# davrempe/caspr

Hardware: AMD Instinct MI355X
Metric: sequences/sec (CaSPR.reconstruct, rigid-cars T=10 N=2048) (higher is better)
Workload: dtype f32 (operands split exactly into 3 bf16, 6 bf16-MFMA partial products per product, f32 accumulate)

## Files before the change

caspr_amd/config.py:

```python
import os
import warnings
from dataclasses import dataclass, asdict


@dataclass
class KernelConfig:
    matmul: str = "bf16x6"
    cnf_split: str = "f16x3"
    cnf_dp5_split: str = "bf16x6"
    conv_split: str = "f16x3"
    emd_route: str = "frame"
    conv_x6w: bool = True
    x6w_min_cin: int = 512
    latent_team: bool = True
    early_latent: bool = True
    early_latent_team: bool = True
    sa_lo_parts: bool = True
    sa_scale_streams: bool = True
    global_stream: bool = True
    sa_pre_aggregate: bool = True
    fp_commute: bool = True
    sa_f64_streams: bool = False
    train_cnf_out_node: bool = True
    train_cnf_hidden_node: bool = True
    train_latent_node: bool = True
    train_cnf_checkpoint: bool = False
    train_cnf_block_node: bool = False


_ENV = {
    "CASPR_MATMUL": ("matmul", lambda v: v.strip().lower()),
    "CASPR_CNF_SPLIT": ("cnf_split", lambda v: v.strip().lower()),
    "CASPR_CNF_DP5_SPLIT": ("cnf_dp5_split", lambda v: v.strip().lower()),
    "CASPR_CONV_SPLIT": ("conv_split", lambda v: v.strip().lower()),
    "CASPR_EMD_ROUTE": ("emd_route", lambda v: v.strip().lower()),
    "CASPR_CONV_X6W": ("conv_x6w", lambda v: v != "0"),
    "CASPR_X6W_MIN_CIN": ("x6w_min_cin", int),
    "CASPR_LATENT_TEAM": ("latent_team", lambda v: v != "0"),
    "CASPR_EARLY_LATENT": (None, None),
    "CASPR_SA_LO_PARTS": ("sa_lo_parts", lambda v: v != "0"),
    "CASPR_SA_SCALE_STREAMS": ("sa_scale_streams", lambda v: v != "0"),
    "CASPR_SA_F64_STREAMS": ("sa_f64_streams", lambda v: v != "0"),
    "CASPR_FP_COMMUTE": ("fp_commute", lambda v: v != "0"),
    "CASPR_SA_PRE_AGGREGATE": ("sa_pre_aggregate", lambda v: v != "0"),
    "CASPR_GLOBAL_STREAM": ("global_stream", lambda v: v != "0"),
    "CASPR_CNF_OUT_NODE": ("train_cnf_out_node", lambda v: v != "0"),
    "CASPR_CNF_NODE": ("train_cnf_hidden_node", lambda v: v != "0"),
    "CASPR_LATENT_NODE": ("train_latent_node", lambda v: v != "0"),
    "CASPR_CNF_CHECKPOINT": ("train_cnf_checkpoint", lambda v: v != "0"),
    "CASPR_CNF_BLOCK_NODE": ("train_cnf_block_node", lambda v: v != "0"),
}


def load(environ=None):
    env = os.environ if environ is None else environ
    cfg = KernelConfig()
    present = [k for k in _ENV if k in env]
    if env.get("CASPR_DEBUG", "0") != "1":
# ... 8 lines not shown
            cfg.early_latent_team = env[name] != "single"
        else:
            setattr(cfg, field, parse(env[name]))
    if cfg.matmul not in ("bf16x6", "f32"):
        raise ValueError("CASPR_MATMUL must be 'bf16x6' or 'f32', got %r" % cfg.matmul)
    if cfg.cnf_split not in ("bf16x6", "f16x3"):
        raise ValueError("CASPR_CNF_SPLIT must be 'bf16x6' or 'f16x3', got %r" % cfg.cnf_split)
    if cfg.cnf_dp5_split not in ("bf16x6", "f16x3"):
        raise ValueError("CASPR_CNF_DP5_SPLIT must be 'bf16x6' or 'f16x3', got %r" % cfg.cnf_dp5_split)
    if cfg.conv_split not in ("bf16x6", "f16x3"):
        raise ValueError("CASPR_CONV_SPLIT must be 'bf16x6' or 'f16x3', got %r" % cfg.conv_split)
    if cfg.emd_route not in ("frame", "rows"):
        raise ValueError("CASPR_EMD_ROUTE must be 'frame' or 'rows', got %r" % cfg.emd_route)
    return cfg


config = load()


def active():
    from . import ops
    from .models import caspr as _c, pointnet2 as _p, tpointnet2 as _t
    d = asdict(config)
    d.update({"matmul": ops.matmul_mode(), "cnf_split": ops.CNF_SPLIT, "cnf_dp5_split": ops.CNF_DP5_SPLIT, "conv_split": ops.CONV_SPLIT, "emd_route": ops.EMD_ROUTE, "conv_x6w": ops.CONV_X6W, "x6w_min_cin": ops._X6W_MIN_CIN, "latent_team": ops.LATENT_TEAM,
              "early_latent": _c.EARLY_LATENT, "early_latent_team": _c.EARLY_LATENT_TEAM, "sa_lo_parts": _p.LO_PARTS,
              "sa_scale_streams": _p.SCALE_STREAMS, "sa_f64_streams": _p.F64_STREAMS, "fp_commute": _p.FP_COMMUTE, "sa_pre_aggregate": _p.PRE_AGGREGATE, "global_stream": _t.GLOBAL_STREAM, "debug_env": os.environ.get("CASPR_DEBUG", "0") == "1"})
    return d
```

caspr_amd/csrc/audit.py:

```python
import os
import re
import subprocess
import tempfile

LLVM = os.environ.get("CASPR_LLVM_BIN", "/opt/rocm/lib/llvm/bin")
TESTED_HIPCC = "HIP version: 7.2.26015-fc0010cf6a / AMD clang version 22.0.0git roc-7.2.0"


class AuditError(RuntimeError):
    pass


def tools_present():
    return all(os.path.exists(os.path.join(LLVM, t)) for t in ("llvm-objdump", "llvm-objcopy", "llvm-readelf", "clang-offload-bundler"))


def _code_object(obj):
    with tempfile.TemporaryDirectory() as d:
        fat, elf = os.path.join(d, "w.fatbin"), os.path.join(d, "w.elf")
        subprocess.check_call([os.path.join(LLVM, "llvm-objcopy"), "--dump-section", ".hip_fatbin=" + fat, obj, os.path.join(d, "copy.o")])
        subprocess.check_call([os.path.join(LLVM, "clang-offload-bundler"), "--unbundle", "--type=o", "--input=" + fat,
                               "--targets=hipv4-amdgcn-amd-amdhsa--gfx950", "--output=" + elf])
        notes = subprocess.check_output([os.path.join(LLVM, "llvm-readelf"), "--notes", elf], text=True)
        dis = subprocess.check_output([os.path.join(LLVM, "llvm-objdump"), "-d", elf], text=True)
# ... 119 lines not shown
        mfma = [i for i in ins if i.startswith("v_mfma")]
        _need(len(mfma) == 2 * 192 and all(re.match(r"v_mfma_f32_32x32x16_bf16 a\[", i) for i in mfma), "%s: %d MFMAs, not all on a[..]" % (k, len(mfma)))
        out.append({"kernel": k, "accvgpr_reads": r, "accvgpr_writes": w, "mfma": len(mfma)})
    return out


def audit_conv_h3w(obj):
    notes, dis = _code_object(obj)
    kernels = re.findall(r"<(_Z18conv1x1_h3w_kernelI[^>]*)>:", dis)
    _need(len(kernels) >= 4, "conv1x1_h3w_kernel: %d instantiations found" % len(kernels))
    out = []
    for k in kernels:
        meta, ins = _kernel(notes, dis, k)
        count = lambda pat: sum(1 for i in ins if re.match(pat, i))
        _no_spills(meta, ins, k)
        r, w = count(r"v_accvgpr_read_b32"), count(r"v_accvgpr_write_b32")
        _need(w == 768 and r == 512 and count(r"v_accvgpr_mov") == 0, "%s: %d reads / %d writes of the accumulator file (512 / 768 in the source)" % (k, r, w))
        mfma = [i for i in ins if i.startswith("v_mfma")]
        _need(len(mfma) == 2 * 96 and all(re.match(r"v_mfma_f32_32x32x16_f16 a\[", i) for i in mfma), "%s: %d MFMAs, not all v_mfma_f32_32x32x16_f16 on a[..]" % (k, len(mfma)))
        out.append({"kernel": k, "accvgpr_reads": r, "accvgpr_writes": w, "mfma": len(mfma), "cvt_pk": count(r"v_cvt_pk_f16_f32")})
    return out


AUDITS = {"ode_bf16x6w.hip": audit_cnf_x6w, "ode_f16x3w.hip": audit_cnf_h3w, "ode_dp5_f16x3w.hip": audit_cnf_dp5_h3w, "gemm_bf16x6w.hip": audit_conv_x6w, "gemm_f16x3w.hip": audit_conv_h3w}


def audit_objects(objs_by_source):
    if not tools_present():
        raise AuditError("the ROCm LLVM tools (%s: llvm-objdump, llvm-objcopy, llvm-readelf, clang-offload-bundler) are needed to audit the "
                         "hand-managed accumulator kernels" % LLVM)
    res = {}
    for src, fn in AUDITS.items():
        if src in objs_by_source:
            try:
                res[src] = fn(objs_by_source[src])
            except (AuditError, ValueError, IndexError, subprocess.CalledProcessError) as e:
                ver = subprocess.run([os.environ.get("HIPCC", "/opt/rocm/bin/hipcc"), "--version"], capture_output=True, text=True).stdout.splitlines()[:2]
                raise AuditError("%s\n  this compiler: %s\n  tested with:   %s\n  -> the library is NOT produced (CASPR_SKIP_AUDIT=1 overrides, "
                                 "see caspr_amd/csrc/audit.py)" % (e, " / ".join(ver), TESTED_HIPCC)) from None
    return res


def audit_no_packed_f32(objs_by_source):
    if not tools_present():
        raise AuditError("the ROCm LLVM tools (%s) are needed to check the objects for packed-f32 instructions" % LLVM)
    res = {}
    for src, obj in sorted(objs_by_source.items()):
# ... 11 lines not shown
```

caspr_amd/csrc/build.py:

```python
import os
import subprocess
import sys
from concurrent.futures import ThreadPoolExecutor

HERE = os.path.dirname(os.path.abspath(__file__))
sys.path.insert(0, os.path.abspath(os.path.join(HERE, "..", "..")))
SOURCES = ["point_ops.hip", "gemm.hip", "gemm_bf16x6.hip", "gemm_bf16x6w.hip", "gemm_f16x3w.hip", "sa_mlp.hip", "ode.hip", "ode_bf16x6.hip", "ode_bf16x6w.hip", "ode_f16x3w.hip", "cnf_frame_steps.hip", "ode_dp5.hip", "ode_dp5_f16x3w.hip", "ode_train_fwd.hip", "ode_sample_tape.hip", "ode_latent_dp5.hip", "backward.hip", "backward_points.hip", "backward_flow.hip", "backward_flow_value.hip", "emd.hip", "emd_exact.hip", "pose.hip", "base_sample.hip"]
EXTRA = {"point_ops.hip": ["-ffp-contract=off"], "emd.hip": ["-ffp-contract=off"], "pose.hip": ["-ffp-contract=off"],
         "emd_exact.hip": ["-ffp-contract=off"],
         "cnf_frame_steps.hip": ["-ffp-contract=off"],
         "base_sample.hip": ["-ffp-contract=off"],
         "ode_bf16x6.hip": ["-mllvm", "-pragma-unroll-threshold=400000"],
         "ode_dp5.hip": ["-mllvm", "-pragma-unroll-threshold=400000"],
         "ode_train_fwd.hip": ["-mllvm", "-pragma-unroll-threshold=400000"],
         "ode_sample_tape.hip": ["-mllvm", "-pragma-unroll-threshold=400000"],
         "ode_bf16x6w.hip": ["-mllvm", "-pragma-unroll-threshold=400000", "-mllvm", "-amdgpu-mfma-vgpr-form", "-fno-slp-vectorize"],
         "ode_f16x3w.hip": ["-mllvm", "-pragma-unroll-threshold=400000", "-mllvm", "-amdgpu-mfma-vgpr-form", "-fno-slp-vectorize"],
         "ode_dp5_f16x3w.hip": ["-mllvm", "-pragma-unroll-threshold=400000", "-mllvm", "-amdgpu-mfma-vgpr-form", "-fno-slp-vectorize"],
         "gemm_bf16x6w.hip": ["-mllvm", "-pragma-unroll-threshold=400000", "-mllvm", "-amdgpu-mfma-vgpr-form", "-fno-slp-vectorize"],
         "gemm_f16x3w.hip": ["-mllvm", "-pragma-unroll-threshold=400000", "-mllvm", "-amdgpu-mfma-vgpr-form", "-fno-slp-vectorize"]}
DEBUG = os.environ.get("CASPR_BUILD_DEBUG", "0") not in ("0", "")
XW_EXP = os.environ.get("CASPR_XW_EXP", "")
DEBUG = DEBUG or bool(XW_EXP)
OUT = os.path.join(HERE, ("libcaspr_hip_debug_xw%s.so" % XW_EXP) if XW_EXP else ("libcaspr_hip_debug.so" if DEBUG else "libcaspr_hip.so"))
HIPCC = os.environ.get("HIPCC", "/opt/rocm/bin/hipcc")
NO_PACKED_F32 = ["-Xclang", "-target-feature", "-Xclang", "-packed-fp32-ops"]
FLAGS = ["--offload-arch=gfx950", "-O3", "-std=c++17", "-fPIC", "-Wall", "-Wno-unused-function"] + NO_PACKED_F32


def _stale(target, deps):
    if not os.path.exists(target):
        return True
    t = os.path.getmtime(target)
    return any(os.path.getmtime(d) > t for d in deps)


def deps():
    inc = os.path.join(HERE, "..", "..", "include")
    return [os.path.abspath(__file__)] + sorted(os.path.join(HERE, f) for f in os.listdir(HERE) if f.endswith((".h", ".inc"))) + sorted(os.path.join(inc, f) for f in os.listdir(inc) if f.endswith(".h"))


def build(force=False, verbose=False):
# ... 41 lines not shown
```

caspr_amd/csrc/gemm_bf16x6.hip:

```cpp
#include "common.h"
#include <type_traits>

typedef short bf16x8 __attribute__((ext_vector_type(8)));
typedef unsigned u32x4 __attribute__((ext_vector_type(4)));

#define X6_TM 256
#define X6_TP 128
#define X6_PA (X6_TM * 64)
#define X6_PB (X6_TP * 64)
#define X6_CHUNK (3 * X6_PA)
#define X6_LDS (3 * X6_PA + 3 * X6_PB)

__device__ __host__ __forceinline__ int x6_swz(int row) { return (row >> 1) & 3; }
__device__ __forceinline__ int x6_off(int row, int piece) { return row * 64 + ((piece ^ x6_swz(row)) << 4); }

__device__ __forceinline__ void x6_split(float x, float &h1, float &h2, float &h3)
{
    h1 = __uint_as_float(__float_as_uint(x) & 0xffff0000u);
    const float r1 = x - h1;
    h2 = __uint_as_float(__float_as_uint(r1) & 0xffff0000u);
    const float r2 = r1 - h2;
    h3 = __uint_as_float(__float_as_uint(r2) & 0xffff0000u);
}
typedef __bf16 x6_bf16x2 __attribute__((ext_vector_type(2)));
// ... 676 lines not shown
                                  X6Act{gate, const_cast<float *>(Z), ldz, (float *)ws});
    if (rc != CASPR_OK) return rc;
    const long tot = (long)frames * Cout;
    cnf_act_bwd_reduce_kernel<<<dim3((unsigned)((tot + 255) / 256)), dim3(256), 0, (hipStream_t)stream>>>((const float *)ws, frames, 2 * n / X6_TP * 2, Cout,
                                                                                                         dgate, dbeta);
    CASPR_CHECK_LAUNCH("conv1x1_cnf_act_bwd");
    return CASPR_OK;
}

extern "C" int caspr_conv1x1_bf16x6_f32(const void *wpk, const float *bias, const float *bbias, const float *X, int ldx,
                                        const float *in_scale, const float *in_shift, int in_relu, int in_relu_from, float *Y,
                                        int ldy, int B, int P, int Cin, int Cout, int act, void *stream)
{
    CASPR_REQUIRE(Y, "conv1x1_bf16x6: Y is NULL");
    return conv_x6_launch(wpk, bias, bbias, X, ldx, in_scale, in_shift, in_relu, in_relu_from, Y, ldy, B, P, Cin, Cout, act, nullptr, stream);
}

extern "C" long caspr_conv_gn_ws_bytes(int B, int P, int Cout)
{
    if (B <= 0 || P <= 0 || Cout <= 0 || P % X6_TP) return 0;
    return (long)B * (P / X6_TP) * Cout * 16;
}

static int conv_gn_x6_impl(const void *wpk, const float *bias, const float *bbias, const float *X, int ldx, const float *in_scale,
                           const float *in_shift, int in_relu, int in_relu_from, float *Y, int ldy, int B, int P, int Cin, int Cout, int G,
                           int pool, const float *gamma, const float *beta, float eps, float *scale, float *shift, float *pmax, float *mean,
                           float *rstd, void *ws, long ws_bytes, void *stream)
{
    CASPR_REQUIRE(gamma && beta && scale && shift && ws && G > 0, "conv1x1_gn_bf16x6: bad arguments");
    CASPR_REQUIRE(Cout % G == 0, "conv1x1_gn_bf16x6: Cout=%d is not a multiple of the %d groups", Cout, G);
    CASPR_REQUIRE((mean == nullptr) == (rstd == nullptr), "conv1x1_gn_bf16x6: mean / rstd must be given together");
    CASPR_REQUIRE(pool >= 1 && B % pool == 0, "conv1x1_gn_bf16x6: pool=%d must divide B=%d", pool, B);
    CASPR_REQUIRE(B <= 65535 * (long)pool, "conv1x1_gn_bf16x6: B too large");
    CASPR_REQUIRE(P % X6_TP == 0 && ws_bytes >= caspr_conv_gn_ws_bytes(B, P, Cout) && ((uintptr_t)ws % 16) == 0,
                  "conv1x1_gn_bf16x6: workspace too small or misaligned (%ld < %ld)", ws_bytes, caspr_conv_gn_ws_bytes(B, P, Cout));
    const int rc = conv_x6_launch(wpk, bias, bbias, X, ldx, in_scale, in_shift, in_relu, in_relu_from, Y, ldy, B, P, Cin, Cout, 0,
                                  (f32x4 *)ws, stream);
    if (rc != CASPR_OK) return rc;
    conv_gn_finalize_kernel<<<dim3(G, B / pool), dim3(256), 0, (hipStream_t)stream>>>((const f32x4 *)ws, pool * (P / X6_TP), pool * P, Cout, G, gamma,
                                                                                      beta, eps, scale, shift, pmax, mean, rstd);
    CASPR_CHECK_LAUNCH("conv1x1_gn_bf16x6");
    return CASPR_OK;
}

extern "C" int caspr_conv1x1_gn_bf16x6_f32(const void *wpk, const float *bias, const float *bbias, const float *X, int ldx,
                                           const float *in_scale, const float *in_shift, int in_relu, int in_relu_from, float *Y,
                                           int ldy, int B, int P, int Cin, int Cout, int G, const float *gamma, const float *beta,
                                           float eps, float *scale, float *shift, float *pmax, float *mean, float *rstd, void *ws,
                                           long ws_bytes, void *stream)
{
    return conv_gn_x6_impl(wpk, bias, bbias, X, ldx, in_scale, in_shift, in_relu, in_relu_from, Y, ldy, B, P, Cin, Cout, G, 1, gamma, beta, eps, scale,
                           shift, pmax, mean, rstd, ws, ws_bytes, stream);
}

extern "C" int caspr_conv1x1_gn_pooled_bf16x6_f32(const void *wpk, const float *bias, const float *bbias, const float *X, int ldx,
                                                  const float *in_scale, const float *in_shift, int in_relu, int in_relu_from, float *Y,
                                                  int ldy, int B, int P, int Cin, int Cout, int G, int pool, const float *gamma,
                                                  const float *beta, float eps, float *scale, float *shift, float *pmax, float *mean,
                                                  float *rstd, void *ws, long ws_bytes, void *stream)
{
// ... 196 lines not shown
```

caspr_amd/lib.py:

```python
import ctypes
import os

_HERE = os.path.dirname(os.path.abspath(__file__))
SO_PATH = os.path.join(_HERE, "csrc", "libcaspr_hip.so")

c_fp = ctypes.c_void_p
c_ip = ctypes.c_void_p
c_int = ctypes.c_int
c_long = ctypes.c_long
c_float = ctypes.c_float
c_stream = ctypes.c_void_p

SIGNATURES = {
    "caspr_last_error_string": (ctypes.c_char_p, []),
    "caspr_abi_version": (c_int, []),
    "caspr_prep_input_f32": (c_int, [c_fp, c_int, c_int, c_int, c_int, c_fp, c_fp, c_stream]),
    "caspr_fps_f32": (c_int, [c_fp, c_int, c_int, c_int, c_int, c_ip, c_fp, c_stream]),
    "caspr_gather_points_f32": (c_int, [c_fp, c_int, c_ip, c_int, c_int, c_int, c_int, c_fp, c_int, c_stream]),
    "caspr_ball_query_f32": (c_int, [c_fp, c_fp, c_int, c_int, c_int, c_float, c_int, c_ip, c_stream]),
    "caspr_ball_query2_f32": (c_int, [c_fp, c_fp, c_int, c_int, c_int, c_float, c_int, c_ip, c_float, c_int, c_ip, c_stream]),
    "caspr_group_points_f32": (c_int, [c_fp, c_fp, c_fp, c_int, c_ip, c_int, c_int, c_int, c_int, c_int, c_fp, c_stream]),
    "caspr_sa_mlp_max_f32": (c_int, [c_fp, c_fp, c_fp, c_int, c_ip, c_int, c_int, c_int, c_int, c_int, c_int,
                                     c_fp, c_fp, c_fp, c_fp, c_int,
                                     c_fp, c_fp, c_fp, c_fp, c_int,
# ... 3 lines not shown
    "caspr_sa_mlp_max_ws_f32": (c_int, [c_fp, c_fp, c_fp, c_int, c_ip, c_int, c_int, c_int, c_int, c_int, c_int,
                                        c_fp, c_fp, c_fp, c_fp, c_int,
                                        c_fp, c_fp, c_fp, c_fp, c_int,
                                        c_fp, c_fp, c_fp, c_fp, c_int,
                                        c_fp, c_int, c_int, c_ip, c_stream]),
    "caspr_sa_mlp_max_pre_f32": (c_int, [c_fp, c_fp, c_fp, c_int, c_ip, c_int, c_int, c_int, c_int,
                                         c_fp, c_fp, c_fp, c_fp, c_int,
                                         c_fp, c_fp, c_fp, c_fp, c_int,
                                         c_fp, c_fp, c_fp, c_fp, c_int,
                                         c_fp, c_int, c_int, c_stream]),
    "caspr_group_rows_pre_f32": (c_int, [c_fp, c_fp, c_fp, c_int, c_ip, c_int, c_int, c_int, c_int, c_int, c_fp, c_fp, c_fp, c_int, c_stream]),
    "caspr_three_nn_f32": (c_int, [c_fp, c_fp, c_int, c_int, c_int, c_fp, c_ip, c_fp, c_stream]),
    "caspr_three_interp_f32": (c_int, [c_fp, c_int, c_ip, c_fp, c_fp, c_fp, c_int, c_fp, c_int, c_int, c_int, c_int, c_int, c_int, c_fp, c_int, c_stream]),
    "caspr_three_interp_add_gn_ws_bytes": (c_long, [c_int, c_int, c_int]),
    "caspr_three_interp_add_gn_f32": (c_int, [c_fp, c_int, c_ip, c_fp, c_fp, c_int, c_int, c_fp, c_fp, c_int, c_int, c_int, c_int, c_fp, c_int,
                                              c_int, c_fp, c_fp, c_float, c_fp, c_fp, ctypes.c_void_p, c_long, c_stream]),
    "caspr_packed_size": (c_long, [c_int, c_int]),
    "caspr_pack_weight_f32": (c_int, [c_fp, c_int, c_int, c_int, c_int, c_fp, c_stream]),
    "caspr_conv1x1_f32": (c_int, [c_fp, c_fp, c_fp, c_fp, c_int, c_fp, c_fp, c_int, c_int, c_fp, c_int, c_int, c_int, c_int, c_int, c_int, c_stream]),
    "caspr_bf16x3_packed_bytes": (c_long, [c_int, c_int]),
    "caspr_pack_weight_bf16x3": (c_int, [c_fp, c_int, c_int, c_int, c_int, ctypes.c_void_p, c_stream]),
    "caspr_conv1x1_bf16x6_f32": (c_int, [ctypes.c_void_p, c_fp, c_fp, c_fp, c_int, c_fp, c_fp, c_int, c_int, c_fp, c_int, c_int, c_int, c_int, c_int, c_int, c_stream]),
    "caspr_conv_gn_ws_bytes": (c_long, [c_int, c_int, c_int]),
    "caspr_conv1x1_gn_bf16x6_f32": (c_int, [ctypes.c_void_p, c_fp, c_fp, c_fp, c_int, c_fp, c_fp, c_int, c_int, c_fp, c_int, c_int, c_int, c_int, c_int,
                                            c_int, c_fp, c_fp, c_float, c_fp, c_fp, c_fp, c_fp, c_fp, ctypes.c_void_p, c_long, c_stream]),
    "caspr_conv1x1_gn_pooled_bf16x6_f32": (c_int, [ctypes.c_void_p, c_fp, c_fp, c_fp, c_int, c_fp, c_fp, c_int, c_int, c_fp, c_int, c_int, c_int, c_int, c_int,
                                                   c_int, c_int, c_fp, c_fp, c_float, c_fp, c_fp, c_fp, c_fp, c_fp, ctypes.c_void_p, c_long, c_stream]),
    "caspr_x6w_packed_bytes": (c_long, [c_int, c_int]),
    "caspr_pack_weight_x6w": (c_int, [c_fp, c_int, c_int, c_int, c_int, ctypes.c_void_p, c_stream]),
    "caspr_conv1x1_x6w_f32": (c_int, [ctypes.c_void_p, ctypes.c_void_p, c_fp, c_fp, c_fp, c_int, c_fp, c_fp, c_int, c_int, c_fp, c_int, c_int, c_int, c_int,
                                      c_int, c_int, c_fp, c_fp, c_float, c_fp, c_fp, c_fp, c_fp, c_fp, ctypes.c_void_p, c_long, c_stream]),
    "caspr_conv1x1_x6w_pooled_f32": (c_int, [ctypes.c_void_p, ctypes.c_void_p, c_fp, c_fp, c_fp, c_int, c_fp, c_fp, c_int, c_int, c_fp, c_int, c_int, c_int, c_int,
                                             c_int, c_int, c_int, c_fp, c_fp, c_float, c_fp, c_fp, c_fp, c_fp, c_fp, ctypes.c_void_p, c_long, c_stream]),
    "caspr_conv1x1_x6w_part_f32": (c_int, [ctypes.c_void_p, ctypes.c_void_p, c_fp, c_fp, c_fp, c_int, c_fp, c_fp, c_int, c_int, c_fp, c_int, c_int, c_int, c_int,
                                           c_int, c_int, c_int, c_int, c_int, ctypes.c_void_p, c_long, c_stream]),
    "caspr_h3w_packed_bytes": (c_long, [c_int, c_int]),
    "caspr_pack_weight_h3w": (c_int, [c_fp, c_int, c_int, c_int, c_int, ctypes.c_void_p, c_stream]),
    "caspr_conv1x1_h3w_f32": (c_int, [ctypes.c_void_p, ctypes.c_void_p, c_fp, c_fp, c_fp, c_int, c_fp, c_fp, c_int, c_int, c_fp, c_int, c_int, c_int, c_int,
                                      c_int, c_int, c_fp, c_fp, c_float, c_fp, c_fp, c_fp, c_fp, c_fp, ctypes.c_void_p, c_long, ctypes.c_void_p, c_stream]),
    "caspr_conv1x1_h3w_pooled_f32": (c_int, [ctypes.c_void_p, ctypes.c_void_p, c_fp, c_fp, c_fp, c_int, c_fp, c_fp, c_int, c_int, c_fp, c_int, c_int, c_int, c_int,
                                             c_int, c_int, c_int, c_fp, c_fp, c_float, c_fp, c_fp, c_fp, c_fp, c_fp, ctypes.c_void_p, c_long, ctypes.c_void_p,
                                             c_stream]),
    "caspr_conv1x1_h3w_part_f32": (c_int, [ctypes.c_void_p, ctypes.c_void_p, c_fp, c_fp, c_fp, c_int, c_fp, c_fp, c_int, c_int, c_fp, c_int, c_int, c_int, c_int,
                                           c_int, c_int, c_int, c_int, c_int, ctypes.c_void_p, c_long, ctypes.c_void_p, c_stream]),
    "caspr_conv_gn_finalize_f32": (c_int, [ctypes.c_void_p, c_long, c_int, c_int, c_int, c_int, c_int, c_int, c_int, c_fp, c_fp, c_float, c_fp, c_fp, c_fp, c_fp,
                                           c_fp, c_stream]),
# ... 134 lines not shown
```

caspr_amd/ops.py:

```python
import contextlib
import ctypes
import functools

import torch

from . import lib as _lib
from .config import config as _cfg


TIMING = False
TIMERS = {}
TIMING_ONLY = None


class timed:

    def __init__(self, name, level=1):
        self.name = name
        self.level = level

    def __enter__(self):
        self.on = TIMING >= self.level and (TIMING_ONLY is None or TIMING != True or self.name in TIMING_ONLY)
        if self.on:
            self.t0 = torch.cuda.Event(enable_timing=True)
# ... 170 lines not shown
    n = idx.shape[1]
    C = gamma.numel()
    C2 = 0 if skip is None else int(skip_channels)
    y = torch.empty(B, n, C, device=u.device, dtype=torch.float32)
    scale = torch.empty(B, C, device=u.device, dtype=torch.float32)
    shift = torch.empty(B, C, device=u.device, dtype=torch.float32)
    L = _lib.load()
    nb = L.caspr_three_interp_add_gn_ws_bytes(B, n, groups)
    ws = _workspace(nb, u.device)
    with timed("k:three_interp_add_gn:%d:%d:%d" % (C2, C, B * n), 2):
        _lib.check(L.caspr_three_interp_add_gn_f32(_p(u), ldu, _p(idx), _p(weight), _p(skip), lds, C2, _p(wskip), _p(bias), B, m, n, C, _p(y), C,
                                                   groups, _p(gamma), _p(beta), float(eps), _p(scale), _p(shift), _p(ws), ws.numel(), _stream()),
                   "caspr_three_interp_add_gn_f32")
    return y, scale, shift


_mode = _cfg.matmul
CONV_BF16X6 = _mode == "bf16x6"
CONV_X6W = _cfg.conv_x6w
CNF_BF16X6 = _mode == "bf16x6"
CNF_SPLIT = _cfg.cnf_split
CNF_DP5_SPLIT = _cfg.cnf_dp5_split

CONV_SPLIT = _cfg.conv_split


def _split_switch(name):
    value = globals()[name]
    if value not in ("bf16x6", "f16x3"):
        raise ValueError("caspr_amd.ops.%s must be 'bf16x6' or 'f16x3', got %r" % (name, value))
    return value


def conv_split():
    return _split_switch("CONV_SPLIT")


def cnf_dp5_split():
    return _split_switch("CNF_DP5_SPLIT")


def cnf_split():
    return _split_switch("CNF_SPLIT")


_X6_MIN_CIN = 192
# ... 79 lines not shown
        if self._xh is None:
            w2d, ldw, col0, version = self._src
            if w2d._version != version:
                raise RuntimeError("PackedWeight.xh(): the weight tensor was modified in place after this pack was built")
            L = _lib.load()
            cmain = self.cout - self.cout % 512
            main = torch.empty(L.caspr_h3w_packed_bytes(cmain, self.cin), device=w2d.device, dtype=torch.uint8)
            _lib.check(L.caspr_pack_weight_h3w(_p(w2d), ldw, cmain, col0, self.cin, _p(main), _stream()), "caspr_pack_weight_h3w")
            tail = None
            if cmain != self.cout:
                if self._xw is not None:
                    tail = self._xw[1]
                else:
                    wt = w2d[cmain:]
                    tail = torch.empty(L.caspr_bf16x3_packed_bytes(self.cout - cmain, self.cin), device=w2d.device, dtype=torch.uint8)
                    _lib.check(L.caspr_pack_weight_bf16x3(_p(wt), ldw, self.cout - cmain, col0, self.cin, _p(tail), _stream()), "caspr_pack_weight_bf16x3")
            self._xh = (main, tail)
            if self._x3 is not None and self._xw is not None:
                self._src = None
        return self._xh


CONV_ROW_INVARIANT = 0x100


def _pinned(n, dtype):
    return torch.empty(n, dtype=dtype).pin_memory()


def _copy_behind(host, src, stream=None):
    ev = torch.cuda.Event()
    if stream is None:
        host.copy_(src, non_blocking=True)
        ev.record(torch.cuda.current_stream())
    else:
        with torch.cuda.stream(stream):
            host.copy_(src, non_blocking=True)
            ev.record(stream)
    return ev


class _Deferred:
    BACKLOG = 64

    def __init__(self, report):
        self.report = report
# ... 255 lines not shown
    return (y, scale, shift) + (() if mean is None else (mean, rstd)) + (() if pmax is None else (pmax,))


def conv1x1_gn(pw, bias, x, gamma, beta, groups=16, eps=1e-5, want_max=False, want_moments=False, write=True, bbias=None,
               in_scale=None, in_shift=None, in_relu=False, in_relu_from=0, out=None, pool=1, split=None):
    _chk_f32(bias, bbias, in_scale, in_shift, gamma, beta)
    B, P, _ = x.shape
    C = pw.cout
    if pool < 1 or B % pool:
        raise ValueError("conv1x1_gn: pool=%d must divide the %d batch entries" % (pool, B))
    route = _conv_route(pw, B, P, in_relu_from, groups=groups, split=split)
    if route is None:
        y = conv1x1(pw, bias, x, bbias=bbias, in_scale=in_scale, in_shift=in_shift, in_relu=in_relu, in_relu_from=in_relu_from, out=out, split=split)
        yg = y.view(B // pool, pool * P, y.shape[2]) if pool > 1 else y
        if want_moments:
            from . import train_ops
            return (y,) + tuple(train_ops.gn_stats_train(yg, C, gamma, beta, groups, eps, want_max))
        return (y,) + tuple(gn_stats(yg, C, gamma, beta, groups, eps, want_max))
    ldx = _conv_ldx("conv1x1_gn", pw, x)
    y, ldy, scale, shift, mean, rstd, pmax, ws = _conv_gn_buffers(pw, x, pool, groups if want_moments else 0, want_max, out, write)
    if split is None:
        conv_split()
    packs = _conv_wide_packs(route, pw)
    with timed(_conv_timer(route, pw, x), 2):
        _conv_launch(route, "pooled" if pool > 1 else "gn", pw, packs, x, _conv_head(pw, bias, bbias, x, ldx, in_scale, in_shift, in_relu, in_relu_from, y, ldy),
                     (groups,) + ((int(pool),) if pool > 1 else ()) + (_p(gamma), _p(beta), float(eps), _p(scale), _p(shift), _p(pmax), _p(mean), _p(rstd),
                                                                       _p(ws), ws.numel()))
    return _conv_gn_result(y, scale, shift, mean, rstd, pmax)


def _conv_part(route, pw, packs, x, head, ws, mt0, mt1, with_tail, reserve):
    _conv_launch(route, "part", pw, packs, x, head, (mt0, mt1, int(with_tail), int(reserve), _p(ws), ws.numel()))


def _conv_gn_finalize(ws, x, C, groups, pool, gamma, beta, eps, scale, shift, pmax, g0, g1):
    _lib.check(_lib.load().caspr_conv_gn_finalize_f32(_p(ws), ws.numel(), x.shape[0], x.shape[1], C, groups, g0, g1, int(pool), _p(gamma), _p(beta),
                                                      float(eps), _p(scale), _p(shift), _p(pmax), None, None, _stream()), "caspr_conv_gn_finalize_f32")


def conv1x1_gn_early_ok(pw, B, P, groups, early_channels):
    C = pw.cout
    return bool(_conv_route(pw, B, P) in _CONV_WIDE and C % groups == 0 and C // 512 >= 2 and early_channels <= min(C // groups, 512))


def conv1x1_gn_early(pw, bias, x, gamma, beta, on_early, groups=16, eps=1e-5, in_scale=None, in_shift=None, in_relu=False, in_relu_from=0,
                     reserve_cus=1, tail_stream=None):
    _chk_f32(bias, in_scale, in_shift, gamma, beta)
    B, P, _ = x.shape
# ... 727 lines not shown
```

include/caspr_hip.h:

```cpp
#ifndef CASPR_HIP_H
#define CASPR_HIP_H

#include <stdint.h>

#ifdef __cplusplus
extern "C" {
#endif

#define CASPR_OK 0
#define CASPR_EINVAL (-1)
#define CASPR_ELAUNCH (-2)
#define CASPR_EUNSUP (-3)
#define CASPR_ENOCONV (-4)

const char *caspr_last_error_string(void);
int caspr_abi_version(void);

int caspr_prep_input_f32(const float *x, int BT, int N, int quad, int pairs, float *xyz, float *feat,
                         void *stream);

int caspr_fps_f32(const float *xyz, int B, int n, int M, int guard, int32_t *idx, float *new_xyz,
                  void *stream);

int caspr_gather_points_f32(const float *feat, int ldf, const int32_t *idx, int B, int n, int M, int C,
// ... 44 lines not shown
                           const float *in_scale, const float *in_shift, int in_relu, const float *skip,
                           int lds, int B, int m, int n, int C, int C2, float *out, int ldo, void *stream);
long caspr_three_interp_add_gn_ws_bytes(int B, int n, int G);
int caspr_three_interp_add_gn_f32(const float *u, int ldu, const int32_t *idx, const float *weight, const float *skip, int lds,
                                  int C2, const float *wskip, const float *bias, int B, int m, int n, int C, float *y, int ldy,
                                  int G, const float *gamma, const float *beta, float eps, float *scale, float *shift, void *ws,
                                  long ws_bytes, void *stream);


long caspr_packed_size(int Cout, int Cin);
int caspr_pack_weight_f32(const float *w, int ldw, int Cout, int col0, int ncols, float *packed,
                          void *stream);
#define CASPR_CONV_ROW_INVARIANT 0x100
int caspr_conv1x1_f32(const float *wp, const float *bias, const float *bbias, const float *X, int ldx,
                      const float *in_scale, const float *in_shift, int in_relu, int in_relu_from,
                      float *Y, int ldy, int B, int P, int Cin, int Cout, int act, void *stream);

long caspr_bf16x3_packed_bytes(int Cout, int Cin);
int caspr_pack_weight_bf16x3(const float *w, int ldw, int Cout, int col0, int ncols, void *packed, void *stream);
int caspr_conv1x1_bf16x6_f32(const void *wpk, const float *bias, const float *bbias, const float *X, int ldx,
                             const float *in_scale, const float *in_shift, int in_relu, int in_relu_from,
                             float *Y, int ldy, int B, int P, int Cin, int Cout, int act, void *stream);

long caspr_conv_gn_ws_bytes(int B, int P, int Cout);
int caspr_conv1x1_gn_bf16x6_f32(const void *wpk, const float *bias, const float *bbias, const float *X, int ldx,
                                const float *in_scale, const float *in_shift, int in_relu, int in_relu_from,
                                float *Y, int ldy, int B, int P, int Cin, int Cout, int G, const float *gamma,
                                const float *beta, float eps, float *scale, float *shift, float *pmax, float *mean,
                                float *rstd, void *ws, long ws_bytes, void *stream);
int caspr_conv1x1_gn_pooled_bf16x6_f32(const void *wpk, const float *bias, const float *bbias, const float *X, int ldx,
                                       const float *in_scale, const float *in_shift, int in_relu, int in_relu_from,
                                       float *Y, int ldy, int B, int P, int Cin, int Cout, int G, int pool,
                                       const float *gamma, const float *beta, float eps, float *scale, float *shift,
                                       float *pmax, float *mean, float *rstd, void *ws, long ws_bytes, void *stream);

long caspr_x6w_packed_bytes(int Cout, int Cin);
int caspr_pack_weight_x6w(const float *w, int ldw, int Cout, int col0, int ncols, void *packed, void *stream);
int caspr_conv1x1_x6w_f32(const void *wpk_main, const void *wpk_tail, const float *bias, const float *bbias, const float *X, int ldx,
                          const float *in_scale, const float *in_shift, int in_relu, int in_relu_from, float *Y, int ldy, int B,
                          int P, int Cin, int Cout, int G, const float *gamma, const float *beta, float eps, float *scale,
                          float *shift, float *pmax, float *mean, float *rstd, void *ws, long ws_bytes, void *stream);
int caspr_conv1x1_x6w_pooled_f32(const void *wpk_main, const void *wpk_tail, const float *bias, const float *bbias, const float *X, int ldx,
                                 const float *in_scale, const float *in_shift, int in_relu, int in_relu_from, float *Y, int ldy, int B,
                                 int P, int Cin, int Cout, int G, int pool, const float *gamma, const float *beta, float eps, float *scale,
                                 float *shift, float *pmax, float *mean, float *rstd, void *ws, long ws_bytes, void *stream);

// ... 142 lines not shown
```

Measured before the change: 329.5.

## Add stats-only bf16x6 conv kernel for GroupNorm passes with no output

Adds a dedicated 1x1-conv kernel for the small-Cin (32..128) case. When the conv output Y is not needed and only GroupNorm statistics and the per-channel max are wanted, the kernel computes per-tile moments and extrema directly from the MFMA accumulators. This avoids materialising the output tensor. Weights stay register-resident, X tiles are double-buffered through LDS with a bf16x3 split, and work is distributed across XCDs in runs along P. The cost is a new kernel with more templates to audit, plus possible small numerical differences from the two-pass moment combination.

```diff
diff --git a/caspr_amd/config.py b/caspr_amd/config.py
--- a/caspr_amd/config.py
+++ b/caspr_amd/config.py
@@ -10,6 +10,7 @@
     cnf_dp5_split: str = "bf16x6"
     conv_split: str = "f16x3"
     emd_route: str = "frame"
+    conv_stats_only: bool = True
     conv_x6w: bool = True
     x6w_min_cin: int = 512
     latent_team: bool = True
@@ -34,6 +35,7 @@
     "CASPR_CNF_DP5_SPLIT": ("cnf_dp5_split", lambda v: v.strip().lower()),
     "CASPR_CONV_SPLIT": ("conv_split", lambda v: v.strip().lower()),
     "CASPR_EMD_ROUTE": ("emd_route", lambda v: v.strip().lower()),
+    "CASPR_CONV_STATS_ONLY": ("conv_stats_only", lambda v: v != "0"),
     "CASPR_CONV_X6W": ("conv_x6w", lambda v: v != "0"),
     "CASPR_X6W_MIN_CIN": ("x6w_min_cin", int),
     "CASPR_LATENT_TEAM": ("latent_team", lambda v: v != "0"),
@@ -88,7 +90,7 @@
     from . import ops
     from .models import caspr as _c, pointnet2 as _p, tpointnet2 as _t
     d = asdict(config)
-    d.update({"matmul": ops.matmul_mode(), "cnf_split": ops.CNF_SPLIT, "cnf_dp5_split": ops.CNF_DP5_SPLIT, "conv_split": ops.CONV_SPLIT, "emd_route": ops.EMD_ROUTE, "conv_x6w": ops.CONV_X6W, "x6w_min_cin": ops._X6W_MIN_CIN, "latent_team": ops.LATENT_TEAM,
+    d.update({"matmul": ops.matmul_mode(), "cnf_split": ops.CNF_SPLIT, "cnf_dp5_split": ops.CNF_DP5_SPLIT, "conv_split": ops.CONV_SPLIT, "conv_stats_only": ops.CONV_STATS_ONLY, "emd_route": ops.EMD_ROUTE, "conv_x6w": ops.CONV_X6W, "x6w_min_cin": ops._X6W_MIN_CIN, "latent_team": ops.LATENT_TEAM,
               "early_latent": _c.EARLY_LATENT, "early_latent_team": _c.EARLY_LATENT_TEAM, "sa_lo_parts": _p.LO_PARTS,
               "sa_scale_streams": _p.SCALE_STREAMS, "sa_f64_streams": _p.F64_STREAMS, "fp_commute": _p.FP_COMMUTE, "sa_pre_aggregate": _p.PRE_AGGREGATE, "global_stream": _t.GLOBAL_STREAM, "debug_env": os.environ.get("CASPR_DEBUG", "0") == "1"})
     return d
diff --git a/caspr_amd/csrc/audit.py b/caspr_amd/csrc/audit.py
--- a/caspr_amd/csrc/audit.py
+++ b/caspr_amd/csrc/audit.py
@@ -165,7 +165,24 @@
     return out
 
 
-AUDITS = {"ode_bf16x6w.hip": audit_cnf_x6w, "ode_f16x3w.hip": audit_cnf_h3w, "ode_dp5_f16x3w.hip": audit_cnf_dp5_h3w, "gemm_bf16x6w.hip": audit_conv_x6w, "gemm_f16x3w.hip": audit_conv_h3w}
+def audit_conv_x6s(obj):
+    notes, dis = _code_object(obj)
+    kernels = re.findall(r"<(_Z18conv1x1_x6s_kernelILi\d[^>]*)>:", dis)
+    _need(len(kernels) == 8, "conv1x1_x6s_kernel: %d instantiations found (8 expected)" % len(kernels))
+    out = []
+    for k in kernels:
+        meta, ins = _kernel(notes, dis, k)
+        _no_spills(meta, ins, k)
+        nk = int(re.match(r"_Z18conv1x1_x6s_kernelILi(\d)", k).group(1))
+        mfma = [i for i in ins if i.startswith("v_mfma")]
+        want = 48 * nk * (2 if nk & 1 else 1)
+        _need(len(mfma) == want and all(i.startswith("v_mfma_f32_32x32x16_bf16 ") for i in mfma), "%s: %d MFMAs (%d expected), not all v_mfma_f32_32x32x16_bf16" % (k, len(mfma), want))
+        out.append({"kernel": k, "mfma": len(mfma)})
+    return out
+
+
+AUDITS = {"ode_bf16x6w.hip": audit_cnf_x6w, "ode_f16x3w.hip": audit_cnf_h3w, "ode_dp5_f16x3w.hip": audit_cnf_dp5_h3w, "gemm_bf16x6w.hip": audit_conv_x6w, "gemm_f16x3w.hip": audit_conv_h3w,
+          "gemm_bf16x6s.hip": audit_conv_x6s}
 
 
 def audit_objects(objs_by_source):
diff --git a/caspr_amd/csrc/build.py b/caspr_amd/csrc/build.py
--- a/caspr_amd/csrc/build.py
+++ b/caspr_amd/csrc/build.py
@@ -5,7 +5,7 @@
 
 HERE = os.path.dirname(os.path.abspath(__file__))
 sys.path.insert(0, os.path.abspath(os.path.join(HERE, "..", "..")))
-SOURCES = ["point_ops.hip", "gemm.hip", "gemm_bf16x6.hip", "gemm_bf16x6w.hip", "gemm_f16x3w.hip", "sa_mlp.hip", "ode.hip", "ode_bf16x6.hip", "ode_bf16x6w.hip", "ode_f16x3w.hip", "cnf_frame_steps.hip", "ode_dp5.hip", "ode_dp5_f16x3w.hip", "ode_train_fwd.hip", "ode_sample_tape.hip", "ode_latent_dp5.hip", "backward.hip", "backward_points.hip", "backward_flow.hip", "backward_flow_value.hip", "emd.hip", "emd_exact.hip", "pose.hip", "base_sample.hip"]
+SOURCES = ["point_ops.hip", "gemm.hip", "gemm_bf16x6.hip", "gemm_bf16x6s.hip", "gemm_bf16x6w.hip", "gemm_f16x3w.hip", "sa_mlp.hip", "ode.hip", "ode_bf16x6.hip", "ode_bf16x6w.hip", "ode_f16x3w.hip", "cnf_frame_steps.hip", "ode_dp5.hip", "ode_dp5_f16x3w.hip", "ode_train_fwd.hip", "ode_sample_tape.hip", "ode_latent_dp5.hip", "backward.hip", "backward_points.hip", "backward_flow.hip", "backward_flow_value.hip", "emd.hip", "emd_exact.hip", "pose.hip", "base_sample.hip"]
 EXTRA = {"point_ops.hip": ["-ffp-contract=off"], "emd.hip": ["-ffp-contract=off"], "pose.hip": ["-ffp-contract=off"],
          "emd_exact.hip": ["-ffp-contract=off"],
          "cnf_frame_steps.hip": ["-ffp-contract=off"],
@@ -18,6 +18,7 @@
          "ode_f16x3w.hip": ["-mllvm", "-pragma-unroll-threshold=400000", "-mllvm", "-amdgpu-mfma-vgpr-form", "-fno-slp-vectorize"],
          "ode_dp5_f16x3w.hip": ["-mllvm", "-pragma-unroll-threshold=400000", "-mllvm", "-amdgpu-mfma-vgpr-form", "-fno-slp-vectorize"],
          "gemm_bf16x6w.hip": ["-mllvm", "-pragma-unroll-threshold=400000", "-mllvm", "-amdgpu-mfma-vgpr-form", "-fno-slp-vectorize"],
+         "gemm_bf16x6s.hip": ["-mllvm", "-pragma-unroll-threshold=400000", "-fno-slp-vectorize"],
          "gemm_f16x3w.hip": ["-mllvm", "-pragma-unroll-threshold=400000", "-mllvm", "-amdgpu-mfma-vgpr-form", "-fno-slp-vectorize"]}
 DEBUG = os.environ.get("CASPR_BUILD_DEBUG", "0") not in ("0", "")
 XW_EXP = os.environ.get("CASPR_XW_EXP", "")
diff --git a/caspr_amd/csrc/gemm_bf16x6.hip b/caspr_amd/csrc/gemm_bf16x6.hip
--- a/caspr_amd/csrc/gemm_bf16x6.hip
+++ b/caspr_amd/csrc/gemm_bf16x6.hip
@@ -722,6 +722,16 @@
     return (long)B * (P / X6_TP) * Cout * 16;
 }
 
+bool caspr_conv_x6s_ok(int P, int Cin, int Cout) __attribute__((visibility("hidden")));
+int caspr_conv_x6s_launch(const void *wpk, const float *bias, const float *bbias, const float *X, int ldx, const float *in_scale, const float *in_shift,
+                          int in_relu, int in_relu_from, int B, int P, int Cin, int Cout, void *part, int cstride, int runs, hipStream_t stream)
+    __attribute__((visibility("hidden")));
+
+extern "C" int caspr_stats_only_conv_ok(int P, int Cin, int Cout, int has_y, int has_pmax, int in_relu)
+{
+    return !has_y && has_pmax && !(in_relu & CASPR_CONV_GN_TILE_KERNEL) && caspr_conv_x6s_ok(P, Cin, Cout);
+}
+
 static int conv_gn_x6_impl(const void *wpk, const float *bias, const float *bbias, const float *X, int ldx, const float *in_scale,
                            const float *in_shift, int in_relu, int in_relu_from, float *Y, int ldy, int B, int P, int Cin, int Cout, int G,
                            int pool, const float *gamma, const float *beta, float eps, float *scale, float *shift, float *pmax, float *mean,
@@ -734,8 +744,19 @@
     CASPR_REQUIRE(B <= 65535 * (long)pool, "conv1x1_gn_bf16x6: B too large");
     CASPR_REQUIRE(P % X6_TP == 0 && ws_bytes >= caspr_conv_gn_ws_bytes(B, P, Cout) && ((uintptr_t)ws % 16) == 0,
                   "conv1x1_gn_bf16x6: workspace too small or misaligned (%ld < %ld)", ws_bytes, caspr_conv_gn_ws_bytes(B, P, Cout));
-    const int rc = conv_x6_launch(wpk, bias, bbias, X, ldx, in_scale, in_shift, in_relu, in_relu_from, Y, ldy, B, P, Cin, Cout, 0,
-                                  (f32x4 *)ws, stream);
+    const int relu = (in_relu & 0xff) != 0, runs = (in_relu >> CASPR_CONV_GN_RUNS_SHIFT) & 0x7fff;
+    int rc;
+    if (caspr_stats_only_conv_ok(P, Cin, Cout, Y != nullptr, pmax != nullptr, in_relu)) {
+        CASPR_REQUIRE(wpk && X && B > 0, "conv1x1_gn_bf16x6: bad arguments");
+        CASPR_REQUIRE(ldx % 4 == 0 && ldx >= Cin, "conv1x1_bf16x6: ldx=%d must be a multiple of 4 and >= Cin=%d", ldx, Cin);
+        CASPR_REQUIRE((in_scale == nullptr) == (in_shift == nullptr), "conv1x1_bf16x6: in_scale/in_shift must be given together");
+        CASPR_REQUIRE(((uintptr_t)X % 16) == 0 && ((uintptr_t)wpk % 16) == 0 && ((uintptr_t)bias % 16) == 0 && ((uintptr_t)bbias % 16) == 0,
+                      "conv1x1_bf16x6: pointers must be 16-byte aligned");
+        CASPR_REQUIRE(in_relu_from >= 0 && in_relu_from % 8 == 0, "conv1x1_bf16x6: in_relu_from=%d must be a non-negative multiple of 8", in_relu_from);
+        rc = caspr_conv_x6s_launch(wpk, bias, bbias, X, ldx, in_scale, in_shift, relu, in_relu_from, B, P, Cin, Cout, ws, Cout, runs, (hipStream_t)stream);
+    } else {
+        rc = conv_x6_launch(wpk, bias, bbias, X, ldx, in_scale, in_shift, relu, in_relu_from, Y, ldy, B, P, Cin, Cout, 0, (f32x4 *)ws, stream);
+    }
     if (rc != CASPR_OK) return rc;
     conv_gn_finalize_kernel<<<dim3(G, B / pool), dim3(256), 0, (hipStream_t)stream>>>((const f32x4 *)ws, pool * (P / X6_TP), pool * P, Cout, G, gamma,
                                                                                       beta, eps, scale, shift, pmax, mean, rstd);
diff --git a/caspr_amd/csrc/gemm_bf16x6s.hip b/caspr_amd/csrc/gemm_bf16x6s.hip
--- /dev/null
+++ b/caspr_amd/csrc/gemm_bf16x6s.hip
@@ -0,0 +1,256 @@
+#include "x6w_common.h"
+
+#define CS_TP 128
+#define CS_TM 128
+#define CS_FRAG 1024
+#define CS_BCHUNK (2 * 4 * 3 * CS_FRAG)
+#define CS_SPART (2 * CS_BCHUNK)
+#define CS_LDS (2 * CS_BCHUNK + 2 * CS_TM * 16)
+
+#define CS_PK_ROWS 256
+#define CS_PK_PLANE (CS_PK_ROWS * 64)
+#define CS_PK_CHUNK (3 * CS_PK_PLANE)
+__device__ __forceinline__ int cs_pk_off(int row, int piece) { return row * 64 + ((piece ^ ((row >> 1) & 3)) << 4); }
+
+typedef float x6s_f32x2 __attribute__((ext_vector_type(2)));
+
+struct ConvSArgs {
+    const unsigned char *wpk;
+    const float *bias, *bbias, *X;
+    f32x4 *part;
+    int ldx, P, Pt, in_relu, relu_from, nslab, nrun, cstride;
+};
+
+template <int NK, bool FUSED>
+__global__ __launch_bounds__(256, 2) void conv1x1_x6s_kernel(ConvSArgs a, const float *__restrict__ in_scale, const float *__restrict__ in_shift)
+{
+    extern __shared__ __attribute__((aligned(1024))) unsigned char lds[];
+    constexpr int Cin = 32 * NK;
+    const int tid = threadIdx.x, lane = tid & 63;
+    const int wave = __builtin_amdgcn_readfirstlane(tid >> 6);
+    const int nblk = gridDim.x, lin = blockIdx.x;
+    const int xcd = lin & 7, slot = lin >> 3;
+    const int q8 = nblk >> 3, r8 = nblk & 7;
+    const int work = (xcd < r8 ? xcd * (q8 + 1) : r8 * (q8 + 1) + (xcd - r8) * q8) + slot;
+    const int slab = work % a.nslab, run = (work / a.nslab) % a.nrun, b = work / (a.nslab * a.nrun);
+    const int t0 = (int)((long)run * a.Pt / a.nrun), t1 = (int)((long)(run + 1) * a.Pt / a.nrun);
+    const int total = (t1 - t0) * NK;
+
+    bf16x8 wf[2 * NK][3];
+    {
+        const int co = slab * CS_TM + wave * 32 + (lane & 31);
+        const unsigned char *wt = a.wpk + (long)(co / CS_PK_ROWS) * NK * CS_PK_CHUNK;
+        const int row = co % CS_PK_ROWS;
+#pragma unroll
+        for (int ks = 0; ks < 2 * NK; ++ks)
+#pragma unroll
+            for (int pl = 0; pl < 3; ++pl)
+                wf[ks][pl] = *(const bf16x8 *)(wt + (long)(ks >> 1) * CS_PK_CHUNK + pl * CS_PK_PLANE + cs_pk_off(row, 2 * (ks & 1) + (lane >> 5)));
+    }
+    const int cw = slab * CS_TM + wave * 32, hq = (lane >> 5) * 4;
+    f32x4 add[4];
+#pragma unroll
+    for (int rr = 0; rr < 4; ++rr) {
+        add[rr] = (f32x4){0.f, 0.f, 0.f, 0.f};
+        if (a.bias) add[rr] += ld4(a.bias + cw + 8 * rr + hq);
+        if (a.bbias) add[rr] += ld4(a.bbias + (long)b * a.cstride + cw + 8 * rr + hq);
+    }
+
+    const int xr = tid & 127, xh = wave >> 1;
+    const float *xbase = a.X + ((long)b * a.P + xr) * a.ldx + 16 * xh;
+    const unsigned wdst = ((xh * 4 + (xr >> 5)) * 3) * CS_FRAG + (xr & 31) * 16;
+    const float *sc = FUSED ? in_scale + (long)b * Cin + 16 * xh : nullptr;
+    const float *sh = FUSED ? in_shift + (long)b * Cin + 16 * xh : nullptr;
+    f32x4 xreg[4];
+    auto gload = [&](f32x4 (&xv)[4], int g) XW_INL {
+        g = g < total ? g : total - 1;
+        const int t = t0 + g / NK, kc = g % NK;
+        const float *p = xbase + (long)t * CS_TP * a.ldx + kc * 32;
+#pragma unroll
+        for (int q = 0; q < 4; ++q) xv[q] = ld4(p + 4 * q);
+    };
+    auto stage = [&](const f32x4 (&xv)[4], int kc, int buf, int hf) XW_INL {
+        const float lo = (FUSED && a.in_relu && kc * 32 + 16 * xh + 8 * hf >= a.relu_from) ? 0.f : -INFINITY;
+        float v[8];
+#pragma unroll
+        for (int q = 0; q < 8; ++q) {
+            float x = xv[2 * hf + (q >> 2)][q & 3];
+            if (FUSED) {
+                const int k = kc * 32 + 8 * hf + q;
+                x = fmaxf(x * sc[k] + sh[k], lo);
+            }
+            v[q] = x;
+        }
+        u32x4 pv[3];
+#pragma unroll
+        for (int q = 0; q < 4; ++q) {
+            unsigned p1, p2, p3;
+            xc_split_pair(v[2 * q], v[2 * q + 1], p1, p2, p3);
+            pv[0][q] = p1;
+            pv[1][q] = p2;
+            pv[2][q] = p3;
+        }
+#pragma unroll
+        for (int pl = 0; pl < 3; ++pl) *(u32x4 *)(lds + buf * CS_BCHUNK + wdst + pl * CS_FRAG + hf * 512) = pv[pl];
+    };
+    bf16x8 bfr[2][3];
+    auto bread = [&](bf16x8 (&bf)[2][3], int buf, int ct) XW_INL {
+#pragma unroll
+        for (int ks = 0; ks < 2; ++ks)
+#pragma unroll
+            for (int pl = 0; pl < 3; ++pl) bf[ks][pl] = *(const bf16x8 *)(lds + buf * CS_BCHUNK + ((ks * 4 + ct) * 3 + pl) * CS_FRAG + lane * 16);
+    };
+
+    f32x16 acc[4];
+#pragma unroll
+    for (int ct = 0; ct < 4; ++ct)
+#pragma unroll
+        for (int r = 0; r < 16; ++r) acc[ct][r] = 0.f;
+
+    float *spart = (float *)(lds + CS_SPART);
+    const int up = (lane >> 4) & 1;
+    auto moments = [&](auto HFC, auto I0C, auto I1C) XW_INL {
+        constexpr int hf = decltype(HFC)::value;
+        xw_for<decltype(I0C)::value, decltype(I1C)::value>([&](auto IC) XW_INL {
+            constexpr int i = decltype(IC)::value, ra = 2 * i, rb = 2 * i + 1;
+            float x0 = acc[2 * hf][ra] + add[ra >> 2][ra & 3], x1 = acc[2 * hf][rb] + add[rb >> 2][rb & 3];
+            float x2 = acc[2 * hf + 1][ra] + add[ra >> 2][ra & 3], x3 = acc[2 * hf + 1][rb] + add[rb >> 2][rb & 3];
+            xw_swap16(x0, x1);
+            xw_swap16(x2, x3);
+            const float v[4] = {x0, x1, x2, x3};
+            float s1 = 0.f, q1 = 0.f;
+#pragma unroll
+            for (int ni = 0; ni < 4; ++ni) s1 += v[ni];
+            s1 = row_allreduce_add<16>(s1) * (1.0f / 64.0f);
+#pragma unroll
+            for (int ni = 0; ni < 4; ++ni) {
+                const float d = v[ni] - s1;
+                q1 += d * d;
+            }
+            q1 = row_allreduce_add<16>(q1);
+            const int r = 2 * i + up;
+            *(x6s_f32x2 *)(spart + (hf * CS_TM + wave * 32 + (r & 3) + 8 * (r >> 2) + hq) * 4) = (x6s_f32x2){s1, q1};
+        });
+    };
+    auto extrema = [&](auto HFC) XW_INL {
+        constexpr int hf = decltype(HFC)::value;
+        float mx[16], mn[16], mx2[2], mn2[2];
+#pragma unroll
+        for (int r = 0; r < 16; ++r) {
+            const float v0 = acc[2 * hf][r] + add[r >> 2][r & 3], v1 = acc[2 * hf + 1][r] + add[r >> 2][r & 3];
+            mx[r] = fmaxf(v0, v1);
+            mn[r] = fminf(v0, v1);
+            acc[2 * hf][r] = 0.f;
+            acc[2 * hf + 1][r] = 0.f;
+        }
+        xw_treduce16(mx, mx2, XwMax{});
+        xw_treduce16(mn, mn2, XwMin{});
+        const int bk = (lane >> 2) & 3;
+#pragma unroll
+        for (int i = 0; i < 2; ++i) {
+            const int r = 8 * i + 4 * (bk & 1) + 2 * (bk >> 1) + up;
+            *(x6s_f32x2 *)(spart + (hf * CS_TM + wave * 32 + (r & 3) + 8 * (r >> 2) + hq) * 4 + 2) = (x6s_f32x2){mx2[i], mn2[i]};
+        }
+    };
+    auto finish = [&](int t) XW_INL {
+        if (tid < CS_TM) {
+            const f32x4 a0 = ((const f32x4 *)spart)[tid], a1 = ((const f32x4 *)spart)[CS_TM + tid];
+            const float dm = a1[0] - a0[0];
+            a.part[((long)b * a.Pt + t) * a.cstride + slab * CS_TM + tid] =
+                (f32x4){0.5f * (a0[0] + a1[0]), a0[1] + a1[1] + dm * dm * 32.0f, fmaxf(a0[2], a1[2]), fminf(a0[3], a1[3])};
+        }
+        if constexpr (NK == 1) __syncthreads();
+    };
+
+    constexpr int TA[6] = {2, 1, 0, 1, 0, 0}, TB[6] = {0, 1, 2, 0, 1, 0};
+    auto region = [&](auto KCC, auto CTC) XW_INL {
+        constexpr int kc = decltype(KCC)::value, ct = decltype(CTC)::value;
+#pragma unroll
+        for (int i = 0; i < 6; ++i)
+#pragma unroll
+            for (int ks = 0; ks < 2; ++ks) acc[ct] = __builtin_amdgcn_mfma_f32_32x32x16_bf16(wf[2 * kc + ks][TA[i]], bfr[ks][TB[i]], acc[ct], 0, 0, 0);
+    };
+    using I0 = std::integral_constant<int, 0>;
+    using I1 = std::integral_constant<int, 1>;
+    auto chunk = [&](int g, auto KCC, auto CURC) XW_INL {
+        constexpr int kc = decltype(KCC)::value, cur = decltype(CURC)::value, nxt = cur ^ 1;
+        bread(bfr, cur, 0);
+        stage(xreg, (kc + 1) % NK, nxt, 0);
+        region(KCC, I0{});
+        bread(bfr, cur, 1);
+        stage(xreg, (kc + 1) % NK, nxt, 1);
+        region(KCC, I1{});
+        bread(bfr, cur, 2);
+        gload(xreg, g + 2);
+        region(KCC, std::integral_constant<int, 2>{});
+        bread(bfr, cur, 3);
+        region(KCC, std::integral_constant<int, 3>{});
+        if constexpr (kc == NK - 1) {
+            moments(I0{}, I0{}, std::integral_constant<int, 8>{});
+            extrema(I0{});
+            moments(I1{}, I0{}, std::integral_constant<int, 8>{});
+            extrema(I1{});
+        }
+        __syncthreads();
+    };
+    auto tiles = [&](int g, int t, bool two) XW_INL {
+        xw_for<0, NK>([&](auto KC) XW_INL { chunk(g + decltype(KC)::value, KC, std::integral_constant<int, (decltype(KC)::value & 1)>{}); });
+        finish(t);
+        if constexpr (NK & 1) {
+            if (two) {
+                xw_for<0, NK>([&](auto KC) XW_INL { chunk(g + NK + decltype(KC)::value, KC, std::integral_constant<int, ((NK + decltype(KC)::value) & 1)>{}); });
+                finish(t + 1);
+            }
+        }
+    };
+
+    gload(xreg, 0);
+    stage(xreg, 0, 0, 0);
+    stage(xreg, 0, 0, 1);
+    gload(xreg, 1);
+    __syncthreads();
+    constexpr int NP = (NK & 1) ? 2 : 1;
+#pragma unroll 1
+    for (int t = t0; t < t1; t += NP) tiles((t - t0) * NK, t, t + 1 < t1);
+}
+
+bool caspr_conv_x6s_ok(int P, int Cin, int Cout) __attribute__((visibility("hidden")));
+bool caspr_conv_x6s_ok(int P, int Cin, int Cout) { return Cin % 32 == 0 && Cin >= 32 && Cin <= 128 && Cout > 0 && Cout % CS_TM == 0 && P > 0 && P % CS_TP == 0; }
+
+int caspr_conv_x6s_launch(const void *wpk, const float *bias, const float *bbias, const float *X, int ldx, const float *in_scale, const float *in_shift,
+                          int in_relu, int in_relu_from, int B, int P, int Cin, int Cout, void *part, int cstride, int runs, hipStream_t stream)
+    __attribute__((visibility("hidden")));
+
+int caspr_conv_x6s_launch(const void *wpk, const float *bias, const float *bbias, const float *X, int ldx, const float *in_scale, const float *in_shift,
+                          int in_relu, int in_relu_from, int B, int P, int Cin, int Cout, void *part, int cstride, int runs, hipStream_t stream)
+{
+    CASPR_REQUIRE(wpk && X && part && B > 0 && caspr_conv_x6s_ok(P, Cin, Cout), "conv1x1_bf16x6s: bad arguments (Cin=%d Cout=%d P=%d)", Cin, Cout, P);
+    ConvSArgs a;
+    a.wpk = (const unsigned char *)wpk; a.bias = bias; a.bbias = bbias; a.X = X; a.part = (f32x4 *)part;
+    a.ldx = ldx; a.P = P; a.Pt = P / CS_TP; a.in_relu = in_relu; a.relu_from = in_relu_from; a.nslab = Cout / CS_TM; a.cstride = cstride;
+    static int n_cu = 0;
+    if (!n_cu) {
+        int dev = 0, v = 0;
+        (void)hipGetDevice(&dev);
+        n_cu = (hipDeviceGetAttribute(&v, hipDeviceAttributeMultiprocessorCount, dev) == hipSuccess && v > 0) ? v : 256;
+    }
+    const long base = (long)a.nslab * B;
+    long nrun = runs > 0 ? runs : 2L * n_cu / base;
+    nrun = nrun < 1 ? 1 : (nrun > a.Pt ? a.Pt : nrun);
+    a.nrun = (int)nrun;
+    const long nblk = base * nrun;
+    CASPR_REQUIRE(nblk < (1L << 31), "conv1x1_bf16x6s: too many workgroups (%ld)", nblk);
+    const bool fused = in_scale != nullptr;
+#define CS_GO(NK, F) conv1x1_x6s_kernel<NK, F><<<dim3((unsigned)nblk), dim3(256), CS_LDS, stream>>>(a, in_scale, in_shift)
+#define CS_GO_NK(NK) do { if (fused) CS_GO(NK, true); else CS_GO(NK, false); } while (0)
+    switch (Cin / 32) {
+    case 1: CS_GO_NK(1); break;
+    case 2: CS_GO_NK(2); break;
+    case 3: CS_GO_NK(3); break;
+    default: CS_GO_NK(4); break;
+    }
+#undef CS_GO_NK
+#undef CS_GO
+    CASPR_CHECK_LAUNCH("conv1x1_bf16x6s");
+    return CASPR_OK;
+}
diff --git a/caspr_amd/lib.py b/caspr_amd/lib.py
--- a/caspr_amd/lib.py
+++ b/caspr_amd/lib.py
@@ -49,6 +49,7 @@
     "caspr_pack_weight_bf16x3": (c_int, [c_fp, c_int, c_int, c_int, c_int, ctypes.c_void_p, c_stream]),
     "caspr_conv1x1_bf16x6_f32": (c_int, [ctypes.c_void_p, c_fp, c_fp, c_fp, c_int, c_fp, c_fp, c_int, c_int, c_fp, c_int, c_int, c_int, c_int, c_int, c_int, c_stream]),
     "caspr_conv_gn_ws_bytes": (c_long, [c_int, c_int, c_int]),
+    "caspr_stats_only_conv_ok": (c_int, [c_int, c_int, c_int, c_int, c_int, c_int]),
     "caspr_conv1x1_gn_bf16x6_f32": (c_int, [ctypes.c_void_p, c_fp, c_fp, c_fp, c_int, c_fp, c_fp, c_int, c_int, c_fp, c_int, c_int, c_int, c_int, c_int,
                                             c_int, c_fp, c_fp, c_float, c_fp, c_fp, c_fp, c_fp, c_fp, ctypes.c_void_p, c_long, c_stream]),
     "caspr_conv1x1_gn_pooled_bf16x6_f32": (c_int, [ctypes.c_void_p, c_fp, c_fp, c_fp, c_int, c_fp, c_fp, c_int, c_int, c_fp, c_int, c_int, c_int, c_int, c_int,
diff --git a/caspr_amd/ops.py b/caspr_amd/ops.py
--- a/caspr_amd/ops.py
+++ b/caspr_amd/ops.py
@@ -216,6 +216,8 @@
 CNF_SPLIT = _cfg.cnf_split
 CNF_DP5_SPLIT = _cfg.cnf_dp5_split
 
+CONV_STATS_ONLY = _cfg.conv_stats_only
+CONV_STATS_RUNS = 0
 CONV_SPLIT = _cfg.conv_split
 
 
@@ -341,6 +343,8 @@
 
 
 CONV_ROW_INVARIANT = 0x100
+CONV_GN_TILE_KERNEL = 0x100
+CONV_GN_RUNS_SHIFT = 16
 
 
 def _pinned(n, dtype):
@@ -642,8 +646,11 @@
     if split is None:
         conv_split()
     packs = _conv_wide_packs(route, pw)
+    relu = int(bool(in_relu))
+    if route == "x6" and y is None:
+        relu |= (0 if CONV_STATS_ONLY and split is None else CONV_GN_TILE_KERNEL) | (int(CONV_STATS_RUNS) << CONV_GN_RUNS_SHIFT)
     with timed(_conv_timer(route, pw, x), 2):
-        _conv_launch(route, "pooled" if pool > 1 else "gn", pw, packs, x, _conv_head(pw, bias, bbias, x, ldx, in_scale, in_shift, in_relu, in_relu_from, y, ldy),
+        _conv_launch(route, "pooled" if pool > 1 else "gn", pw, packs, x, _conv_head(pw, bias, bbias, x, ldx, in_scale, in_shift, relu, in_relu_from, y, ldy),
                      (groups,) + ((int(pool),) if pool > 1 else ()) + (_p(gamma), _p(beta), float(eps), _p(scale), _p(shift), _p(pmax), _p(mean), _p(rstd),
                                                                        _p(ws), ws.numel()))
     return _conv_gn_result(y, scale, shift, mean, rstd, pmax)
diff --git a/include/caspr_hip.h b/include/caspr_hip.h
--- a/include/caspr_hip.h
+++ b/include/caspr_hip.h
@@ -90,6 +90,9 @@
                              const float *in_scale, const float *in_shift, int in_relu, int in_relu_from,
                              float *Y, int ldy, int B, int P, int Cin, int Cout, int act, void *stream);
 
+#define CASPR_CONV_GN_TILE_KERNEL 0x100
+#define CASPR_CONV_GN_RUNS_SHIFT 16
+int caspr_stats_only_conv_ok(int P, int Cin, int Cout, int has_y, int has_pmax, int in_relu);
 long caspr_conv_gn_ws_bytes(int B, int P, int Cout);
 int caspr_conv1x1_gn_bf16x6_f32(const void *wpk, const float *bias, const float *bbias, const float *X, int ldx,
                                 const float *in_scale, const float *in_shift, int in_relu, int in_relu_from,
```

New measurement: 329.4. Within noise of the previous version (-0.0%).
